# yangsenwxy/VSR

Measured on AMD Instinct MI355X. Metric: voxels/sec fwd+bwd, 4× SR on 16×128×128 cine volumes, 1/2/4/8 MI355X, higher is better.
Workload: dtype bf16

## Files before the change

### vsr_amd/csrc/conv_row.hip

```cpp
#include <cstdlib>
#include "conv_common.h"

namespace {
using namespace vsrk_conv;

constexpr int CR_NW = 8;
constexpr int CR_SEG = 128;
constexpr int CR_SLOT = (CR_SEG + 2) * 128;
constexpr int CR_NSLOT = 4;
constexpr int CR_BIAS = CR_NSLOT * CR_SLOT;
constexpr int CR_LDS = CR_BIAS + 256;
constexpr int CR_MINBAND = 4;
constexpr uint32_t CR_OOB = 0x80000000u;
enum { CE_RES = 1, CE_MASK = 2, CE_ACC = 4, CE_RELU = 8 };

typedef __amdgpu_buffer_rsrc_t CrRsrc;
typedef int cr_v4i __attribute__((ext_vector_type(4)));
__device__ __forceinline__ CrRsrc cr_rsrc(const void* base) {
  const uint64_t b = (uint64_t)base;
  const uint64_t u = ((uint64_t)(uint32_t)__builtin_amdgcn_readfirstlane((int)(uint32_t)(b >> 32)) << 32) |
                     (uint32_t)__builtin_amdgcn_readfirstlane((int)(uint32_t)b);
  return __builtin_amdgcn_make_buffer_rsrc((void*)u, 0, 0x7FFFFFF0, 0x00020000);
}
__device__ __forceinline__ uint4 cr_load16(CrRsrc r, uint32_t voff, uint32_t soff) {
  return __builtin_bit_cast(uint4, __builtin_amdgcn_raw_buffer_load_b128(r, (int)voff, (int)soff, 0));
}
__device__ __forceinline__ void cr_store16(CrRsrc r, uint32_t voff, uint4 v) {
  __builtin_amdgcn_raw_buffer_store_b128(__builtin_bit_cast(cr_v4i, v), r, (int)voff, 0, 0);
}

struct CrView {
  const char* ptr;
  int64_t sn, sd;
  int sh, sw;
};

struct ConvRowArgs {
  CrView x, y, res, msk;
  const void* w;
  const float* bias;
  int cout_pad, cin_pad;
  float out_scale;
  int D, H, W;
  int nseg, nband, band_h, nitems;
};

template <int EM, bool HALO, typename H>
__global__ __launch_bounds__(CR_NW * 64, 1) void conv_row_kernel(ConvRowArgs a) {
  extern __shared__ __attribute__((aligned(16))) char lds[];
  const int tid = threadIdx.x, lane = tid & 63, r = lane & 31, hf = lane >> 5;
  const int wave = __builtin_amdgcn_readfirstlane(tid >> 6);
  const int coh = wave & 1, vq = wave >> 1;

  uint4 wf[9][4];
  {
    const H* wp = reinterpret_cast<const H*>(a.w);
#pragma unroll
    for (int t = 0; t < 9; ++t)
#pragma unroll
      for (int c = 0; c < 4; ++c)
        wf[t][c] = *reinterpret_cast<const uint4*>(wp + ((int64_t)(t * a.cout_pad + coh * 32 + r) * a.cin_pad + c * 16 + 8 * hf));
  }
  const int ecc = 2 * (r >> 4) + hf;
  const int ech = coh * 32 + 8 * ecc;
  const float osc = a.out_scale;
  float* lbias = reinterpret_cast<float*>(lds + CR_BIAS);
  if (tid < 64) lbias[tid] = a.bias ? a.bias[tid] * osc : 0.f;
  if constexpr (!HALO) {
    if (tid < CR_NSLOT * 16)
      *reinterpret_cast<uint4*>(lds + (tid >> 4) * CR_SLOT + ((tid >> 3) & 1) * (CR_SEG + 1) * 128 + (tid & 7) * 16) =
          make_uint4(0, 0, 0, 0);
  }

  uint32_t fa[3], fh[3];
#pragma unroll
  for (int kw = 0; kw < 3; ++kw) {
    const int lv = vq * 32 + r + kw, sz = (lv >> 1) & 7;
    fa[kw] = (uint32_t)(lv * 128 + ((hf ^ (sz & 1)) << 4));
    fh[kw] = (uint32_t)(sz >> 1);
  }
  const int sp = lane & 7;
  constexpr int NSQ = HALO ? 3 : 2;
  const int scol = 8 * wave + (lane >> 3);
  const int hcol = (lane >> 3) == 0 ? -1 : CR_SEG;
  const uint32_t sdst = (uint32_t)((scol + 1) * 128 + ((sp ^ (((scol + 1) >> 1) & 7)) << 4));
  const uint32_t hdst = (uint32_t)((hcol + 1) * 128 + ((sp ^ (((hcol + 1) >> 1) & 7)) << 4));
  const bool halo_lane = wave == 0 && lane < 16;

  f32x16 b0, b1;

  for (int item = blockIdx.x; item < a.nitems; item += gridDim.x) {
    const int band = item % a.nband;
    const int t1 = item / a.nband;
    const int seg = t1 % a.nseg, img = t1 / a.nseg;
    const int in_ = img / a.D, id = img - in_ * a.D;
    const int c0 = seg * CR_SEG;
    const int r0 = band * a.band_h, r1 = min(r0 + a.band_h, a.H);
    const int nstage = r1 - r0 + 1;

    const CrRsrc rx = cr_rsrc(reinterpret_cast<const H*>(a.x.ptr) + (in_ * a.x.sn + id * a.x.sd));
    const CrRsrc ry = cr_rsrc(reinterpret_cast<const H*>(a.y.ptr) + (in_ * a.y.sn + id * a.y.sd));
    const CrRsrc rr = cr_rsrc(reinterpret_cast<const H*>(a.res.ptr) + (in_ * a.res.sn + id * a.res.sd));
    const CrRsrc rm = cr_rsrc(reinterpret_cast<const H*>(a.msk.ptr) + (in_ * a.msk.sn + id * a.msk.sd));

    const uint32_t xcolb = 2u * (uint32_t)((c0 + scol) * a.x.sw + 8 * sp);
    const uint32_t hcolb = 2u * (uint32_t)((c0 + hcol) * a.x.sw + 8 * sp);
    bool xok[3];
    xok[0] = c0 + scol < a.W;
    xok[1] = c0 + scol + 64 < a.W;
    xok[2] = halo_lane && c0 + hcol >= 0 && c0 + hcol < a.W;
    const int ecol = c0 + vq * 32 + (r & 15);
    const uint32_t ycolb = 2u * (uint32_t)(ecol * a.y.sw + ech);
    const uint32_t rcolb = 2u * (uint32_t)(ecol * a.res.sw + ech);
    const uint32_t mcolb = 2u * (uint32_t)(ecol * a.msk.sw + ech);
    const bool yok[2] = {ecol < a.W, ecol + 16 < a.W};

    uint4 stq[CR_NSLOT][NSQ];
    auto load_row = [&](int row, uint4 (&st)[NSQ]) __attribute__((always_inline)) {
      const bool rv = row >= 0 && row < a.H && row <= r1;
      const uint32_t rb = rv ? 2u * (uint32_t)(row * a.x.sh) : 0u;
#pragma unroll
      for (int q = 0; q < 2; ++q) st[q] = cr_load16(rx, (rv && xok[q]) ? xcolb : CR_OOB, rb + 2u * (uint32_t)(64 * q * a.x.sw));
      if constexpr (HALO) st[2] = cr_load16(rx, (rv && xok[2]) ? hcolb : CR_OOB, rb);
    };
    auto write_row = [&](int slot, const uint4 (&st)[NSQ]) __attribute__((always_inline)) {
      char* sl = lds + slot * CR_SLOT;
#pragma unroll
      for (int q = 0; q < 2; ++q) *reinterpret_cast<uint4*>(sl + sdst + q * 64 * 128) = st[q];
      if constexpr (HALO) {
        if (halo_lane) *reinterpret_cast<uint4*>(sl + hdst) = st[NSQ - 1];
      }
    };

    uint4 pr[2], pm[2], po[2];
    auto load_pre = [&](int orow) __attribute__((always_inline)) {
      const bool rv = orow >= r0 && orow < r1;
#pragma unroll
      for (int q = 0; q < 2; ++q) {
        const bool ok = rv && yok[q];
        const int ro = rv ? orow : 0;
        if constexpr (EM & CE_RES) pr[q] = cr_load16(rr, ok ? rcolb : CR_OOB, 2u * (uint32_t)(ro * a.res.sh + 16 * q * a.res.sw));
        if constexpr (EM & CE_MASK) pm[q] = cr_load16(rm, ok ? mcolb : CR_OOB, 2u * (uint32_t)(ro * a.msk.sh + 16 * q * a.msk.sw));
        if constexpr (EM & CE_ACC) po[q] = cr_load16(ry, ok ? ycolb : CR_OOB, 2u * (uint32_t)(ro * a.y.sh + 16 * q * a.y.sw));
      }
    };

    auto flush = [&](const f32x16& A, int orow) __attribute__((always_inline)) {
      const bool rv = orow >= r0 && orow < r1;
      float v[16];
#pragma unroll
      for (int i = 0; i < 16; ++i) v[i] = A[i];
#pragma unroll
      for (int g = 0; g < 4; g += 2) {
#pragma unroll
        for (int i = 0; i < 4; ++i) {
          const auto sw = __builtin_amdgcn_permlane32_swap(__builtin_bit_cast(uint32_t, v[4 * g + i]),
                                                           __builtin_bit_cast(uint32_t, v[4 * g + 4 + i]), false, false);
          v[4 * g + i] = __builtin_bit_cast(float, (uint32_t)sw[0]);
          v[4 * g + 4 + i] = __builtin_bit_cast(float, (uint32_t)sw[1]);
        }
      }
#pragma unroll
      for (int e = 0; e < 8; ++e) {
        const auto sw = __builtin_amdgcn_permlane16_swap(__builtin_bit_cast(uint32_t, v[e]),
                                                         __builtin_bit_cast(uint32_t, v[8 + e]), false, false);
        v[e] = __builtin_bit_cast(float, (uint32_t)sw[0]);
        v[8 + e] = __builtin_bit_cast(float, (uint32_t)sw[1]);
      }
      float bsv[8];
      {
        const float4 c0 = *reinterpret_cast<const float4*>(lbias + ech);
        const float4 c1 = *reinterpret_cast<const float4*>(lbias + ech + 4);
        bsv[0] = c0.x; bsv[1] = c0.y; bsv[2] = c0.z; bsv[3] = c0.w;
        bsv[4] = c1.x; bsv[5] = c1.y; bsv[6] = c1.z; bsv[7] = c1.w;
      }
#pragma unroll
      for (int q = 0; q < 2; ++q) {
        float t[8];
#pragma unroll
        for (int e = 0; e < 8; ++e) {
          t[e] = fmaf(v[8 * q + e], osc, bsv[e]);
          if constexpr (EM & CE_RELU) t[e] = fmaxf(t[e], 0.f);
        }
        if constexpr (EM & CE_MASK) {
          float m[8];
          Chunk<H>::unpack(pm[q], m);
#pragma unroll
          for (int e = 0; e < 8; ++e) t[e] = m[e] > 0.f ? t[e] : 0.f;
        }
        if constexpr (EM & CE_RES) {
          float rs[8];
          Chunk<H>::unpack(pr[q], rs);
#pragma unroll
          for (int e = 0; e < 8; ++e) t[e] += rs[e];
        }
        if constexpr (EM & CE_ACC) {
          float o[8];
          Chunk<H>::unpack(po[q], o);
#pragma unroll
          for (int e = 0; e < 8; ++e) t[e] += o[e];
        }
        const uint32_t yo = ycolb + 2u * (uint32_t)((rv ? orow : 0) * a.y.sh + 16 * q * a.y.sw);
        cr_store16(ry, (rv && yok[q]) ? yo : CR_OOB, Chunk<H>::pack(t));
      }
    };

    __syncthreads();
    load_row(r0 - 1, stq[0]);
    load_row(r0, stq[1]);
    load_row(r0 + 1, stq[2]);
    load_row(r0 + 2, stq[3]);
    write_row(0, stq[0]);
    write_row(1, stq[1]);
    write_row(2, stq[2]);
    load_pre(r0 - 1);

    int s = 0;
    auto step = [&](auto k_c, f32x16& Pcur, const f32x16& Pprev) __attribute__((always_inline)) -> bool {
      constexpr int K = decltype(k_c)::value;
      const int o = r0 + s;
      __syncthreads();
      load_row(o + 3, stq[K]);
      flush(Pprev, o - 1);
      load_pre(o);
#pragma unroll
      for (int kw = 0; kw < 3; ++kw) asm volatile("" : "+v"(fh[kw]));
#pragma unroll
      for (int c = 0; c < 4; ++c) {
#pragma unroll
        for (int kw = 0; kw < 3; ++kw) {
          const uint32_t fo = fa[kw] + (((uint32_t)c ^ fh[kw]) << 5);
#pragma unroll
          for (int kh = 0; kh < 3; ++kh) {
            const uint4 f = *reinterpret_cast<const uint4*>(lds + ((K + kh) % CR_NSLOT) * CR_SLOT + fo);
            if (c == 0 && kw == 0 && kh == 0) {
#pragma unroll
              for (int k = 0; k < 16; ++k) Pcur[k] = 0.f;
            }
            mma<H>(Pcur, wf[kh * 3 + kw][c], f);
          }
        }
      }
      write_row((K + 3) % CR_NSLOT, stq[(K + 3) % CR_NSLOT]);
      return ++s < nstage;
    };
#pragma unroll
    for (int k = 0; k < 16; ++k) b0[k] = b1[k] = 0.f;
    while (step(std::integral_constant<int, 0>{}, b0, b1) && step(std::integral_constant<int, 1>{}, b1, b0) &&
           step(std::integral_constant<int, 2>{}, b0, b1) && step(std::integral_constant<int, 3>{}, b1, b0)) {
    }
  }
}

unsigned long long g_row_launches = 0;

int cr_env_mode() {
  const char* e = getenv("VSRK_CONV_ROW");
  return !e ? -1 : (e[0] == '0' ? 0 : 1);
}
const int g_row_env = cr_env_mode();
int g_row_mode = g_row_env;

int cr_num_cus() {
  static int n = 0;
  if (n == 0) {
    int dev = 0;
    (void)hipGetDevice(&dev);
    if (hipDeviceGetAttribute(&n, hipDeviceAttributeMultiprocessorCount, dev) != hipSuccess || n <= 0) n = 256;
  }
  return n;
}

template <int EM, typename H>
int launch_row(const ConvRowArgs& a, int grid, hipStream_t s) {
  auto kern = a.nseg > 1 ? conv_row_kernel<EM, true, H> : conv_row_kernel<EM, false, H>;
  (void)hipFuncSetAttribute((const void*)kern, hipFuncAttributeMaxDynamicSharedMemorySize, CR_LDS);
  kern<<<grid, CR_NW * 64, CR_LDS, s>>>(a);
  ++g_row_launches;
  VSRK_LAUNCH_CHECK("conv_fwd(row)");
  return VSRK_OK;
}

constexpr bool cr_default_on(int em) {
  return em == 0 || em == CE_RELU || em == CE_RES || em == CE_MASK || em == (CE_RES | CE_ACC);
}

}

extern "C" unsigned long long vsrk_conv_row_launches(void) { return g_row_launches; }

void vsrk_conv_set_row_mode(int mode) { g_row_mode = mode < 0 ? g_row_env : mode; }

int vsrk_conv_fwd_row(const vsrk_conv_desc* d, const vsrk_tensor5* x, const void* w_packed, const float* bias,
                      const vsrk_tensor5* residual, const vsrk_tensor5* mask, const vsrk_tensor5* y, hipStream_t s) {
  if (g_row_mode == 0) return 0;
  if (d->kd != 1 || d->kh != 3 || d->kw != 3 || d->pd != 0 || d->ph != 1 || d->pw != 1) return 0;
  if (x->c != 64 || y->c != 64 || x->shuffle > 1 || y->shuffle > 1) return 0;
  if (d->prologue || d->mask_slope || d->bias_perm_r > 1 || d->subpixel) return 0;
  if (d->act != VSRK_ACT_NONE && d->act != VSRK_ACT_RELU) return 0;
  if (x->n != y->n || x->d != y->d || x->h != y->h || x->w != y->w) return 0;
  const int em = (residual ? CE_RES : 0) | (mask ? CE_MASK : 0) | (d->accumulate ? CE_ACC : 0) |
                 (d->act == VSRK_ACT_RELU ? CE_RELU : 0);
  if (em != 0 && em != CE_RELU && em != CE_RES && em != CE_MASK && em != (CE_RES | CE_ACC)) return 0;
  if (g_row_mode < 0 && !cr_default_on(em)) return 0;
  if (!chunk_ok(x, 2)) return 0;
  for (const vsrk_tensor5* t : {x, y, residual, mask}) {
    if (!t) continue;
    const int64_t span = (int64_t)(t->h - 1) * t->sh + (int64_t)(t->w - 1) * t->sw + 64;
    if (t->sn < 0 || t->sd < 0 || t->sh < 0 || t->sw < 0 || 2 * span >= 0x7FFFFFF0ll) return 0;
    if (t->sh >= (1ll << 30) || t->sw >= (1ll << 30)) return 0;
  }
  const int64_t nimg = (int64_t)y->n * y->d;
  if (nimg == 0 || y->h == 0 || y->w == 0) return 1;
  auto view = [](const vsrk_tensor5* t) {
    CrView v;
    v.ptr = (const char*)t->ptr;
    v.sn = t->sn; v.sd = t->sd; v.sh = (int)t->sh; v.sw = (int)t->sw;
    return v;
  };
  ConvRowArgs a;
  a.x = view(x);
  a.y = view(y);
  a.res = view(residual ? residual : y);
  a.msk = view(mask ? mask : y);
  a.w = w_packed;
  a.bias = bias;
  a.cin_pad = round_up(x->c, 32);
  a.cout_pad = round_up(y->c, 128);
  a.out_scale = d->out_scale;
  a.D = y->d; a.H = y->h; a.W = y->w;
  a.nseg = ceil_div(y->w, CR_SEG);
  const int64_t target = vsrk_capped_grid(cr_num_cus());
  const int64_t cols = nimg * a.nseg;
  int64_t nb = std::max<int64_t>(1, std::min<int64_t>(ceil_div64(target, cols), y->h));
  a.band_h = (int)std::max<int64_t>(ceil_div64(y->h, nb), std::min(CR_MINBAND, y->h));
  a.nband = ceil_div(y->h, a.band_h);
  const int64_t nitems = cols * a.nband;
  if (nitems >= (1ll << 31)) return 0;
  a.nitems = (int)nitems;
  const int grid = (int)vsrk_capped_grid(std::min<int64_t>(nitems, cr_num_cus()));
  int rc = vsrk_dispatch16(x->dtype, [&](auto tag) {
    using H = decltype(tag);
    switch (em) {
      case 0: return launch_row<0, H>(a, grid, s);
      case CE_RELU: return launch_row<CE_RELU, H>(a, grid, s);
      case CE_RES: return launch_row<CE_RES, H>(a, grid, s);
      case CE_MASK: return launch_row<CE_MASK, H>(a, grid, s);
      default: return launch_row<CE_RES | CE_ACC, H>(a, grid, s);
    }
  });
  return rc == VSRK_OK ? 1 : -rc;
}
```

### vsr_amd/csrc/conv_wgrad_row.hip

```cpp
#include <algorithm>
#include <cstdlib>
#include "conv_common.h"

namespace {
using namespace vsrk_conv;

constexpr int RW_NW = 8;
constexpr int RW_KC = 4;
constexpr int RW_SEG = 32 * RW_KC;
constexpr int RW_XV = RW_SEG + 8;
constexpr int RW_XP = RW_XV / 8;
constexpr int RW_YP = RW_SEG / 8;
constexpr int RW_NP = RW_XP + RW_YP;
constexpr int RW_NQ = (RW_NP + RW_NW - 1) / RW_NW;
constexpr int RW_XSLOT = RW_XP * 1024;
constexpr int RW_YSLOT = RW_YP * 1024;
constexpr int RW_NXS = 4, RW_NYS = 2;
constexpr int RW_YBASE = RW_NXS * RW_XSLOT;
constexpr int RW_LDS = RW_YBASE + RW_NYS * RW_YSLOT;
constexpr int RW_COW = 64;
constexpr int RW_SLAB = 9 * RW_COW * 64 + RW_COW;
constexpr uint32_t RW_OOB = 0x80000000u;

#ifndef RW_ABL
#define RW_ABL 0
#endif

__host__ __device__ constexpr int rw_swz(int j) { return 2 * ((j >> 1) & 1) + 4 * ((j >> 3) & 1); }

typedef __amdgpu_buffer_rsrc_t RwRsrc;
__device__ __forceinline__ RwRsrc rw_rsrc(const void* base) {
  const uint64_t b = (uint64_t)base;
  const uint64_t u = ((uint64_t)(uint32_t)__builtin_amdgcn_readfirstlane((int)(uint32_t)(b >> 32)) << 32) |
                     (uint32_t)__builtin_amdgcn_readfirstlane((int)(uint32_t)b);
  return __builtin_amdgcn_make_buffer_rsrc((void*)u, 0, 0x7FFFFFF0, 0x00020000);
}
typedef uint32_t rw_u32x4 __attribute__((ext_vector_type(4)));
__device__ __forceinline__ void rw_st16(uint32_t addr, uint4 v) {
  *(__attribute__((address_space(3))) rw_u32x4*)(size_t)addr = __builtin_bit_cast(rw_u32x4, v);
}

typedef float f32x4_t __attribute__((ext_vector_type(4)));
template <typename H> struct V8R;
template <> struct V8R<bf16> { typedef bf16x8 type; };
template <> struct V8R<f16> { typedef f16x8 type; };
__device__ __forceinline__ f32x4_t rw_mfma(bf16x8 a, bf16x8 b, f32x4_t c) {
  return __builtin_amdgcn_mfma_f32_16x16x32_bf16(a, b, c, 0, 0, 0);
}
__device__ __forceinline__ f32x4_t rw_mfma(f16x8 a, f16x8 b, f32x4_t c) {
  return __builtin_amdgcn_mfma_f32_16x16x32_f16(a, b, c, 0, 0, 0);
}
__device__ __forceinline__ uint4 rw_frag(uint32_t p0, uint32_t p1) {
  const v4i16 a = __builtin_amdgcn_ds_read_tr16_b64_v4i16((lds_v4i16*)(size_t)p0);
  const v4i16 b = __builtin_amdgcn_ds_read_tr16_b64_v4i16((lds_v4i16*)(size_t)p1);
  return __builtin_bit_cast(uint4, __builtin_shufflevector(a, b, 0, 1, 2, 3, 4, 5, 6, 7));
}

constexpr int RW_MAXB = 16;

struct RowArgs {
  const char* x;
  const char* dy;
  int xoff[RW_MAXB], yoff[RW_MAXB];
  uint16_t tapm[RW_MAXB];
  int tapm_x;
  float* ws;
  int64_t xsn, xsd, xsh, xsw, ysn, ysd, ysh, ysw;
  int xd, H, W;
  int bands, band_h, nseg, ncot, ncic, nsplit;
  int want_bias;
  int prio;
};

template <typename H, bool SPM>
__global__ __launch_bounds__(RW_NW * 64, 1) void wgrad_row_kernel(RowArgs a) {
  using V8 = typename V8R<H>::type;
  extern __shared__ __attribute__((aligned(16))) char lds[];
  const int lane = threadIdx.x & 63;
  const int wave = __builtin_amdgcn_readfirstlane(threadIdx.x >> 6);
  const int coh = wave & 1, cib = wave >> 1;

  const int ncombo = a.ncot * a.ncic;
  const int L = xcd_remap(blockIdx.x, a.nsplit * ncombo);
  const int split = L / ncombo;
  const int combo = L - split * ncombo;
  const int cot = combo % a.ncot, cic = combo / a.ncot;
  const int seg = split % a.nseg;
  const int t0 = split / a.nseg;
  const int band = t0 % a.bands, img = t0 / a.bands;
  const int nb = img / a.xd, dd = img - nb * a.xd;
  const int h0 = band * a.band_h;
  const int nst = min(a.H, h0 + a.band_h) - h0;
  const int w0 = seg * RW_SEG;
  const unsigned tapm = SPM ? (unsigned)a.tapm[a.tapm_x ? cic : cot] : 0x1ffu;
  const char* xim = a.x + 2 * (nb * a.xsn + dd * a.xsd + a.xoff[cic]);
  const char* yim = a.dy + 2 * (nb * a.ysn + dd * a.ysd + a.yoff[cot]);

  static_assert(RW_XP == 2 * RW_NW + 1 && RW_YP == 2 * RW_NW, "piece roles");
  uint32_t goff[RW_NQ], loff[RW_NQ];
#pragma unroll
  for (int q = 0; q < RW_NQ; ++q) {
    const bool isx = q != 2 && q != 3;
    const int j = q == 4 ? 2 * RW_NW : wave + RW_NW * (q & 1);
    if (isx) {
      const int v = 8 * j + (lane >> 3);
      const int col = w0 - 1 + v;
      const bool ok = v < RW_SEG + 2 && col >= 0 && col < a.W;
      goff[q] = ok ? (uint32_t)(2 * (col * (int)a.xsw + 8 * (lane & 7))) : RW_OOB;
      loff[q] = (uint32_t)(j * 1024 + (lane >> 3) * 128 + 16 * ((lane & 7) ^ rw_swz(v)));
    } else {
      const int v = 8 * j + (lane >> 3);
      const int col = w0 + v;
      goff[q] = col < a.W ? (uint32_t)(2 * (col * (int)a.ysw + 8 * (lane & 7))) : RW_OOB;
      loff[q] = (uint32_t)(j * 1024 + (lane >> 3) * 128 + 16 * ((lane & 7) ^ rw_swz(v)));
    }
  }
  const uint32_t lbase = lds_addr(lds);
  auto load_set = [&](int t, uint4 (&r)[RW_NQ]) __attribute__((always_inline)) {
    const int xr = h0 - 1 + t;
    const bool xok = xr >= 0 && xr < a.H;
    const int yr = t - 2;
    const bool yok = yr >= 0 && yr < nst;
    const RwRsrc rx = rw_rsrc(xim + 2 * (int64_t)(xok ? xr : 0) * a.xsh);
    const RwRsrc ry = rw_rsrc(yim + 2 * (int64_t)(h0 + (yok ? yr : 0)) * a.ysh);
#pragma unroll
    for (int q = 0; q < RW_NQ; ++q) {
      const bool isx = q != 2 && q != 3;
      if (q == 4 && wave != 0) break;
      r[q] = __builtin_bit_cast(uint4, __builtin_amdgcn_raw_buffer_load_b128(
                                           isx ? rx : ry, (int)((isx ? xok : yok) ? goff[q] : RW_OOB), 0, 0));
    }
  };
  auto store_set = [&](int t, const uint4 (&r)[RW_NQ]) __attribute__((always_inline)) {
    const uint32_t xs = lbase + (uint32_t)(t % RW_NXS) * RW_XSLOT;
    const int yr = t - 2;
    const uint32_t ys = lbase + RW_YBASE + (uint32_t)((yr < 0 ? 0 : yr) % RW_NYS) * RW_YSLOT;
#pragma unroll
    for (int q = 0; q < RW_NQ; ++q) {
      const bool isx = q != 2 && q != 3;
      if (q == 4 && wave != 0) break;
      if (isx) rw_st16(xs + loff[q], r[q]);
      else if (yr >= 0) rw_st16(ys + loff[q], r[q]);
    }
  };

  const int g = lane >> 4, qq = (lane >> 2) & 3, pp = lane & 3;
  uint32_t xo[3][2];
#pragma unroll
  for (int kw = 0; kw < 3; ++kw)
#pragma unroll
    for (int h = 0; h < 2; ++h) {
      const int v = kw + 8 * g + qq + 4 * h;
      xo[kw][h] = (uint32_t)(v * 128 + 16 * ((2 * cib + (pp >> 1)) ^ rw_swz(v)) + 8 * (pp & 1));
    }
  uint32_t yo[2][2];
#pragma unroll
  for (int b = 0; b < 2; ++b)
#pragma unroll
    for (int h = 0; h < 2; ++h) {
      const int v = 8 * g + qq + 4 * h;
      yo[b][h] = (uint32_t)(v * 128 + 16 * ((2 * (2 * coh + b) + (pp >> 1)) ^ rw_swz(v)) + 8 * (pp & 1));
    }

  f32x4_t acc[3][3][2];
#pragma unroll
  for (int i = 0; i < 18; ++i) acc[i / 6][(i / 2) % 3][i % 2] = f32x4_t{0.f, 0.f, 0.f, 0.f};
  f32x4_t bacc[2] = {f32x4_t{0.f, 0.f, 0.f, 0.f}, f32x4_t{0.f, 0.f, 0.f, 0.f}};
  uint4 ones;
  {
    const H one = from_f32<H>(1.f);
    const uint16_t u = __builtin_bit_cast(uint16_t, one);
    const uint32_t w2 = (uint32_t)u | ((uint32_t)u << 16);
    ones = make_uint4(w2, w2, w2, w2);
  }

  const int last = nst + 1;
  uint4 stg[RW_NQ], stg2[RW_NQ];
  load_set(0, stg);
  if (1 <= last) load_set(1, stg2);
  store_set(0, stg);
  if (1 <= last) store_set(1, stg2);
  if (2 <= last) {
    load_set(2, stg);
    store_set(2, stg);
  }
  __syncthreads();
  if (3 <= last) load_set(3, stg);
  __builtin_amdgcn_sched_barrier(0);

  for (int s = 0; s < nst; ++s) {
    uint32_t xa[3][3][2], ya[2][2];
#pragma unroll
    for (int kh = 0; kh < 3; ++kh) {
      const uint32_t xrow = lbase + (uint32_t)((s + kh) % RW_NXS) * RW_XSLOT;
#pragma unroll
      for (int kw = 0; kw < 3; ++kw)
#pragma unroll
        for (int h = 0; h < 2; ++h) {
          xa[kh][kw][h] = xrow + xo[kw][h];
          asm volatile("" : "+v"(xa[kh][kw][h]));
        }
    }
    {
      const uint32_t yr = lbase + RW_YBASE + (uint32_t)(s % RW_NYS) * RW_YSLOT;
#pragma unroll
      for (int b = 0; b < 2; ++b)
#pragma unroll
        for (int h = 0; h < 2; ++h) {
          ya[b][h] = yr + yo[b][h];
          asm volatile("" : "+v"(ya[b][h]));
        }
    }
    uint4 xf[2][3], yf[2][2];
    auto load_group = [&](int G) __attribute__((always_inline)) {
      const int kc = G / 3, kh = G % 3;
      if (kh == 0) {
#pragma unroll
        for (int b = 0; b < 2; ++b) yf[kc & 1][b] = rw_frag(ya[b][0] + kc * 4096, ya[b][1] + kc * 4096);
      }
#pragma unroll
      for (int kw = 0; kw < 3; ++kw) xf[G & 1][kw] = rw_frag(xa[kh][kw][0] + kc * 4096, xa[kh][kw][1] + kc * 4096);
    };
    load_group(0);
#pragma unroll
    for (int G = 0; G < 3 * RW_KC; ++G) {
      if (G + 1 < 3 * RW_KC) load_group(G + 1);
      __builtin_amdgcn_sched_barrier(0);
      if (a.prio) __builtin_amdgcn_s_setprio(1);
      const int kc = G / 3, kh = G % 3;
#pragma unroll
      for (int kw = 0; kw < 3; ++kw) {
        if (SPM && !((tapm >> (kh * 3 + kw)) & 1)) continue;
#pragma unroll
        for (int b = 0; b < 2; ++b)
          if (RW_ABL & 2) acc[kh][kw][b][0] += __builtin_bit_cast(float, yf[kc & 1][b].x ^ xf[G & 1][kw].y);
          else acc[kh][kw][b] = rw_mfma(__builtin_bit_cast(V8, yf[kc & 1][b]), __builtin_bit_cast(V8, xf[G & 1][kw]),
                                   acc[kh][kw][b]);
      }
      if (kh == 1 && kc == cib) {
#pragma unroll
        for (int b = 0; b < 2; ++b)
          bacc[b] = rw_mfma(__builtin_bit_cast(V8, yf[kc & 1][b]), __builtin_bit_cast(V8, ones), bacc[b]);
      }
      if (a.prio) __builtin_amdgcn_s_setprio(0);
      __builtin_amdgcn_sched_barrier(0);
    }
    if (!(RW_ABL & 1)) {
      if (s + 3 <= last) store_set(s + 3, stg);
      asm volatile("s_waitcnt lgkmcnt(0)\n\ts_barrier" ::: "memory");
      if (s + 4 <= last) load_set(s + 4, stg);
    }
    __builtin_amdgcn_sched_barrier(0);
  }

  float* out = a.ws + ((int64_t)split * ncombo + combo) * RW_SLAB;
  const int l15 = lane & 15, lg = lane >> 4;
#pragma unroll
  for (int t9 = 0; t9 < 9; ++t9)
#pragma unroll
    for (int b = 0; b < 2; ++b)
#pragma unroll
      for (int i = 0; i < 4; ++i) {
        const int co = 32 * coh + 16 * b + 4 * lg + i, ci = 16 * cib + l15;
        out[(t9 * RW_COW + co) * 64 + ci] = ((tapm >> t9) & 1) ? acc[t9 / 3][t9 % 3][b][i] : 0.f;
      }
  if (a.want_bias && cic == 0) {
    float* part = reinterpret_cast<float*>(lds);
    __syncthreads();
    if (l15 == 0) {
#pragma unroll
      for (int b = 0; b < 2; ++b)
#pragma unroll
        for (int i = 0; i < 4; ++i) part[cib * 64 + 32 * coh + 16 * b + 4 * lg + i] = bacc[b][i];
    }
    __syncthreads();
    if (threadIdx.x < RW_COW) {
      const int c = threadIdx.x;
      out[9 * RW_COW * 64 + c] = ((part[c] + part[64 + c]) + part[128 + c]) + part[192 + c];
    }
  }
}

int g_wrow_mode = -1;

int wrow_num_cus() {
  static int n = 0;
  if (n == 0) {
    int dev = 0;
    (void)hipGetDevice(&dev);
    if (hipDeviceGetAttribute(&n, hipDeviceAttributeMultiprocessorCount, dev) != hipSuccess || n <= 0) n = 256;
  }
  return n;
}

}

void vsrk_conv_set_wgrad_row_mode(int mode) { g_wrow_mode = mode; }

bool vsrk_wgrad_row_plan(const vsrk_conv_desc* d, const vsrk_tensor5* x, const vsrk_tensor5* dy, VsrkRowPlan* p) {
  if (g_wrow_mode < 0) {
    const char* e = getenv("VSRK_WGRAD_ROW");
    g_wrow_mode = (e && e[0] == '0') ? 0 : 1;
  }
  if (g_wrow_mode == 0) return false;
  if (!vsrk_is16(x->dtype) || dy->dtype != x->dtype) return false;
  if (d->kd != 1 || d->kh != 3 || d->kw != 3 || d->pd != 0 || d->ph != 1 || d->pw != 1) return false;
  if (d->prologue != VSRK_PRO_NONE) return false;
  if (x->c % 64 || dy->c % 64 || (x->shuffle > 1 && dy->shuffle > 1)) return false;
  if (d->subpixel && (x->shuffle > 1 || dy->shuffle > 1) && g_wrow_mode != 2) return false;
  if (x->c / 64 > RW_MAXB || dy->c / 64 > RW_MAXB) return false;
  for (const vsrk_tensor5* t : {x, dy}) {
    if (t->shuffle <= 1) continue;
    const int r = t->shuffle, cph = t->c / (r * r);
    if (cph * r * r != t->c || cph % 64) return false;
  }
  if (x->n != dy->n || x->d != dy->d || x->h != dy->h || x->w != dy->w) return false;
  if (!chunk_ok(x, 2) || !chunk_ok(dy, 2)) return false;
  for (const vsrk_tensor5* t : {x, dy}) {
    const int64_t r = t->shuffle > 1 ? t->shuffle : 1;
    if (t->sn < 0 || t->sd < 0 || t->sh < 0 || t->sw < 0 ||
        (int64_t)(RW_XV + 2) * r * t->sw + (r - 1) * t->sh + t->c >= (1ll << 29))
      return false;
  }
  const int64_t images = (int64_t)x->n * x->d;
  if (images <= 0 || x->h <= 0 || x->w <= 0) return false;
  const int nseg = ceil_div(x->w, RW_SEG);
  const int ncot = dy->c / RW_COW, ncic = x->c / 64;
  const int64_t per_band = images * nseg * ncot * ncic;
  int64_t want = std::max<int64_t>(1, wrow_num_cus());
  if (vsrk_g_grid_cap > 0) want = std::min<int64_t>(want, vsrk_g_grid_cap);
  int bands = (int)std::max<int64_t>(1, std::min<int64_t>((want + per_band / 2) / per_band, ceil_div(x->h, 8)));
  {
    static int ov = -1;
    if (ov < 0) {
      const char* e = getenv("VSRK_WGRAD_ROW_BANDS");
      ov = e ? std::max(0, atoi(e)) : 0;
    }
    if (ov > 0) bands = std::min(ov, x->h);
  }
  if (vsrk_g_grid_cap > 0) bands = std::max(1, std::min(bands, x->h));
  p->band_h = ceil_div(x->h, bands);
  p->bands = ceil_div(x->h, p->band_h);
  p->nseg = nseg;
  p->ncot = ncot;
  p->ncic = ncic;
  const int64_t ns = images * p->bands * nseg;
  if (ns * ncot * ncic >= (1ll << 30)) return false;
  p->nsplit = (int)ns;
  p->cot_w = RW_COW;
  p->slab = RW_SLAB;
  p->ws_bytes = (size_t)ns * ncot * ncic * RW_SLAB * sizeof(float);
  return true;
}

int vsrk_conv_wgrad_row(const vsrk_conv_desc* d, const vsrk_tensor5* x, const vsrk_tensor5* dy, int want_bias,
                        float* ws, size_t ws_bytes, VsrkRowPlan* plan, hipStream_t s) {
  VsrkRowPlan p;
  if (!vsrk_wgrad_row_plan(d, x, dy, &p)) return 0;
  if (ws_bytes < p.ws_bytes) return 0;
  RowArgs a;
  a.x = (const char*)x->ptr;
  a.dy = (const char*)dy->ptr;
  a.ws = ws;
  auto blocks = [](const vsrk_tensor5* t, int64_t& sh, int64_t& sw, int* off) {
    const int r = t->shuffle > 1 ? t->shuffle : 1;
    sh = (int64_t)r * t->sh;
    sw = (int64_t)r * t->sw;
    const int cph = t->c / (r * r);
    for (int b = 0; b < t->c / 64; ++b) {
      const int c = 64 * b, sub = c / cph, cc = c - sub * cph;
      off[b] = (int)((sub / r) * t->sh + (sub % r) * t->sw + cc);
    }
  };
  a.xsn = x->sn; a.xsd = x->sd;
  a.ysn = dy->sn; a.ysd = dy->sd;
  blocks(x, a.xsh, a.xsw, a.xoff);
  blocks(dy, a.ysh, a.ysw, a.yoff);
  const vsrk_tensor5* spt = x->shuffle > 1 ? x : (dy->shuffle > 1 ? dy : nullptr);
  const bool spm = d->subpixel && spt;
  a.tapm_x = spt == x;
  if (spm) {
    const int r = spt->shuffle, cph = spt->c / (r * r);
    const int32_t code = d->subpixel & ~(1 << 25);
    for (int b = 0; b < spt->c / 64; ++b) a.tapm[b] = (uint16_t)subpixel_tapmask(code, r, 64 * b / cph);
  }
  a.xd = x->d;
  a.H = x->h;
  a.W = x->w;
  a.bands = p.bands;
  a.band_h = p.band_h;
  a.nseg = p.nseg;
  a.ncot = p.ncot;
  a.ncic = p.ncic;
  a.nsplit = p.nsplit;
  a.want_bias = want_bias;
  {
    static int prio = -1;
    if (prio < 0) {
      const char* e = getenv("VSRK_WGRAD_ROW_PRIO");
      prio = (e && e[0] == '1') ? 1 : 0;
    }
    a.prio = prio;
  }
  const int grid = p.nsplit * p.ncot * p.ncic;
  vsrk_dispatch16(x->dtype, [&](auto tag) {
    using H = decltype(tag);
    auto kern = spm ? wgrad_row_kernel<H, true> : wgrad_row_kernel<H, false>;
    (void)hipFuncSetAttribute((const void*)kern, hipFuncAttributeMaxDynamicSharedMemorySize, RW_LDS);
    kern<<<grid, RW_NW * 64, RW_LDS, s>>>(a);
    return 0;
  });
  *plan = p;
  return 1;
}
```

Before: 61.82 million.

## Interleave epilogue flush with MFMA groups and prefetch LDS reads one group ahead

Splits the previous row's epilogue (permlane swaps, bias, store) into four parts and interleaves them between groups of MFMA instructions, with sched_barriers, for non-halo, non-residual variants. LDS fragment reads are grouped in threes and issued one group ahead of the MFMAs that consume them, so LDS latency and epilogue work overlap with matrix math. It also adds ROW_ABL ablation macros, which are off by default. The costs are higher register pressure from the extra fragment buffers, and sched_barriers that may block the compiler's own better schedules.

After: 62.12 million (median of 3 runs). No clear change (+0.5%).

```diff
diff --git a/vsr_amd/csrc/conv_row.hip b/vsr_amd/csrc/conv_row.hip
--- a/vsr_amd/csrc/conv_row.hip
+++ b/vsr_amd/csrc/conv_row.hip
@@ -13,6 +13,14 @@
 constexpr int CR_MINBAND = 4;
 constexpr uint32_t CR_OOB = 0x80000000u;
 enum { CE_RES = 1, CE_MASK = 2, CE_ACC = 4, CE_RELU = 8 };
+
+#ifndef ROW_ABL
+#define ROW_ABL 0
+#endif
+
+constexpr int CR_AHEAD = 1;
+constexpr int CR_FLUSH_AT[4] = {0, 2, 4, 6};
+constexpr bool cr_spread(int em, bool halo) { return !halo && (em == 0 || em == CE_RELU); }
 
 typedef __amdgpu_buffer_rsrc_t CrRsrc;
 typedef int cr_v4i __attribute__((ext_vector_type(4)));
@@ -133,49 +141,53 @@
     };
 
     uint4 pr[2], pm[2], po[2];
-    auto load_pre = [&](int orow) __attribute__((always_inline)) {
+    auto load_pre = [&](int orow, int q) __attribute__((always_inline)) {
       const bool rv = orow >= r0 && orow < r1;
-#pragma unroll
-      for (int q = 0; q < 2; ++q) {
-        const bool ok = rv && yok[q];
-        const int ro = rv ? orow : 0;
-        if constexpr (EM & CE_RES) pr[q] = cr_load16(rr, ok ? rcolb : CR_OOB, 2u * (uint32_t)(ro * a.res.sh + 16 * q * a.res.sw));
-        if constexpr (EM & CE_MASK) pm[q] = cr_load16(rm, ok ? mcolb : CR_OOB, 2u * (uint32_t)(ro * a.msk.sh + 16 * q * a.msk.sw));
-        if constexpr (EM & CE_ACC) po[q] = cr_load16(ry, ok ? ycolb : CR_OOB, 2u * (uint32_t)(ro * a.y.sh + 16 * q * a.y.sw));
+      const bool ok = rv && yok[q];
+      const int ro = rv ? orow : 0;
+      if constexpr (EM & CE_RES) pr[q] = cr_load16(rr, ok ? rcolb : CR_OOB, 2u * (uint32_t)(ro * a.res.sh + 16 * q * a.res.sw));
+      if constexpr (EM & CE_MASK) pm[q] = cr_load16(rm, ok ? mcolb : CR_OOB, 2u * (uint32_t)(ro * a.msk.sh + 16 * q * a.msk.sw));
+      if constexpr (EM & CE_ACC) po[q] = cr_load16(ry, ok ? ycolb : CR_OOB, 2u * (uint32_t)(ro * a.y.sh + 16 * q * a.y.sw));
+    };
+
+    auto flush_part = [&](auto part_c, float (&v)[16], float (&bsv)[8], const f32x16& A, int orow)
+                          __attribute__((always_inline)) {
+      constexpr int PART = decltype(part_c)::value;
+      if constexpr ((ROW_ABL & 1) != 0) {
+        if constexpr (PART == 0) {
+#pragma unroll
+          for (int i = 0; i < 16; ++i) asm volatile("" ::"v"(A[i]));
+        }
+        return;
       }
-    };
-
-    auto flush = [&](const f32x16& A, int orow) __attribute__((always_inline)) {
-      const bool rv = orow >= r0 && orow < r1;
-      float v[16];
-#pragma unroll
-      for (int i = 0; i < 16; ++i) v[i] = A[i];
-#pragma unroll
-      for (int g = 0; g < 4; g += 2) {
-#pragma unroll
-        for (int i = 0; i < 4; ++i) {
-          const auto sw = __builtin_amdgcn_permlane32_swap(__builtin_bit_cast(uint32_t, v[4 * g + i]),
-                                                           __builtin_bit_cast(uint32_t, v[4 * g + 4 + i]), false, false);
-          v[4 * g + i] = __builtin_bit_cast(float, (uint32_t)sw[0]);
-          v[4 * g + 4 + i] = __builtin_bit_cast(float, (uint32_t)sw[1]);
-        }
-      }
-#pragma unroll
-      for (int e = 0; e < 8; ++e) {
-        const auto sw = __builtin_amdgcn_permlane16_swap(__builtin_bit_cast(uint32_t, v[e]),
-                                                         __builtin_bit_cast(uint32_t, v[8 + e]), false, false);
-        v[e] = __builtin_bit_cast(float, (uint32_t)sw[0]);
-        v[8 + e] = __builtin_bit_cast(float, (uint32_t)sw[1]);
-      }
-      float bsv[8];
-      {
+      if constexpr (PART == 0) {
+#pragma unroll
+        for (int i = 0; i < 16; ++i) v[i] = A[i];
+#pragma unroll
+        for (int g = 0; g < 4; g += 2) {
+#pragma unroll
+          for (int i = 0; i < 4; ++i) {
+            const auto sw = __builtin_amdgcn_permlane32_swap(__builtin_bit_cast(uint32_t, v[4 * g + i]),
+                                                             __builtin_bit_cast(uint32_t, v[4 * g + 4 + i]), false, false);
+            v[4 * g + i] = __builtin_bit_cast(float, (uint32_t)sw[0]);
+            v[4 * g + 4 + i] = __builtin_bit_cast(float, (uint32_t)sw[1]);
+          }
+        }
+      } else if constexpr (PART == 1) {
+#pragma unroll
+        for (int e = 0; e < 8; ++e) {
+          const auto sw = __builtin_amdgcn_permlane16_swap(__builtin_bit_cast(uint32_t, v[e]),
+                                                           __builtin_bit_cast(uint32_t, v[8 + e]), false, false);
+          v[e] = __builtin_bit_cast(float, (uint32_t)sw[0]);
+          v[8 + e] = __builtin_bit_cast(float, (uint32_t)sw[1]);
+        }
         const float4 c0 = *reinterpret_cast<const float4*>(lbias + ech);
         const float4 c1 = *reinterpret_cast<const float4*>(lbias + ech + 4);
         bsv[0] = c0.x; bsv[1] = c0.y; bsv[2] = c0.z; bsv[3] = c0.w;
         bsv[4] = c1.x; bsv[5] = c1.y; bsv[6] = c1.z; bsv[7] = c1.w;
-      }
-#pragma unroll
-      for (int q = 0; q < 2; ++q) {
+      } else {
+        constexpr int q = PART - 2;
+        const bool rv = orow >= r0 && orow < r1;
         float t[8];
 #pragma unroll
         for (int e = 0; e < 8; ++e) {
@@ -203,6 +215,13 @@
         const uint32_t yo = ycolb + 2u * (uint32_t)((rv ? orow : 0) * a.y.sh + 16 * q * a.y.sw);
         cr_store16(ry, (rv && yok[q]) ? yo : CR_OOB, Chunk<H>::pack(t));
       }
+    };
+    auto flush = [&](const f32x16& A, int orow) __attribute__((always_inline)) {
+      float v[16], bsv[8];
+      flush_part(std::integral_constant<int, 0>{}, v, bsv, A, orow);
+      flush_part(std::integral_constant<int, 1>{}, v, bsv, A, orow);
+      flush_part(std::integral_constant<int, 2>{}, v, bsv, A, orow);
+      flush_part(std::integral_constant<int, 3>{}, v, bsv, A, orow);
     };
 
     __syncthreads();
@@ -213,35 +232,63 @@
     write_row(0, stq[0]);
     write_row(1, stq[1]);
     write_row(2, stq[2]);
-    load_pre(r0 - 1);
+    load_pre(r0 - 1, 0);
+    load_pre(r0 - 1, 1);
 
     int s = 0;
     auto step = [&](auto k_c, f32x16& Pcur, const f32x16& Pprev) __attribute__((always_inline)) -> bool {
       constexpr int K = decltype(k_c)::value;
+      constexpr bool SPREAD = cr_spread(EM, HALO);
+      constexpr int D = SPREAD ? CR_AHEAD : 0, GS = 3, NG = 36 / GS;
       const int o = r0 + s;
       __syncthreads();
-      load_row(o + 3, stq[K]);
-      flush(Pprev, o - 1);
-      load_pre(o);
+      if constexpr (!(ROW_ABL & 4)) load_row(o + 3, stq[K]);
+      float v[16], bsv[8];
+      if constexpr (!SPREAD) {
+        flush(Pprev, o - 1);
+        load_pre(o, 0);
+        load_pre(o, 1);
+      }
 #pragma unroll
       for (int kw = 0; kw < 3; ++kw) asm volatile("" : "+v"(fh[kw]));
-#pragma unroll
-      for (int c = 0; c < 4; ++c) {
-#pragma unroll
-        for (int kw = 0; kw < 3; ++kw) {
+      uint4 fr[D + 1][GS];
+      auto read_group = [&](int g) __attribute__((always_inline)) {
+#pragma unroll
+        for (int j = 0; j < GS; ++j) {
+          const int m = g * GS + j, c = m / 9, kw = (m / 3) % 3, kh = m % 3;
           const uint32_t fo = fa[kw] + (((uint32_t)c ^ fh[kw]) << 5);
-#pragma unroll
-          for (int kh = 0; kh < 3; ++kh) {
-            const uint4 f = *reinterpret_cast<const uint4*>(lds + ((K + kh) % CR_NSLOT) * CR_SLOT + fo);
-            if (c == 0 && kw == 0 && kh == 0) {
-#pragma unroll
-              for (int k = 0; k < 16; ++k) Pcur[k] = 0.f;
-            }
-            mma<H>(Pcur, wf[kh * 3 + kw][c], f);
+          fr[g % (D + 1)][j] = *reinterpret_cast<const uint4*>(lds + ((K + kh) % CR_NSLOT) * CR_SLOT + fo);
+        }
+      };
+#pragma unroll
+      for (int g = 0; g < D; ++g) read_group(g);
+#pragma unroll
+      for (int k = 0; k < 16; ++k) Pcur[k] = 0.f;
+#pragma unroll
+      for (int g = 0; g < NG; ++g) {
+        if (g + D < NG) read_group(g + D);
+        if constexpr (SPREAD) {
+          __builtin_amdgcn_sched_barrier(0);
+          if (g == CR_FLUSH_AT[0]) flush_part(std::integral_constant<int, 0>{}, v, bsv, Pprev, o - 1);
+          if (g == CR_FLUSH_AT[1]) flush_part(std::integral_constant<int, 1>{}, v, bsv, Pprev, o - 1);
+          if (g == CR_FLUSH_AT[2]) {
+            flush_part(std::integral_constant<int, 2>{}, v, bsv, Pprev, o - 1);
+            load_pre(o, 0);
           }
-        }
+          if (g == CR_FLUSH_AT[3]) {
+            flush_part(std::integral_constant<int, 3>{}, v, bsv, Pprev, o - 1);
+            load_pre(o, 1);
+          }
+        }
+#pragma unroll
+        for (int j = 0; j < GS; ++j) {
+          const int m = g * GS + j, c = m / 9, kw = (m / 3) % 3, kh = m % 3;
+          if constexpr ((ROW_ABL & 2) != 0) Pcur[kh] += __builtin_bit_cast(float, fr[g % (D + 1)][j].x ^ wf[kh * 3 + kw][c].y);
+          else mma<H>(Pcur, wf[kh * 3 + kw][c], fr[g % (D + 1)][j]);
+        }
+        if constexpr (SPREAD) __builtin_amdgcn_sched_barrier(0);
       }
-      write_row((K + 3) % CR_NSLOT, stq[(K + 3) % CR_NSLOT]);
+      if constexpr (!(ROW_ABL & 4)) write_row((K + 3) % CR_NSLOT, stq[(K + 3) % CR_NSLOT]);
       return ++s < nstage;
     };
 #pragma unroll
```

## Stagger conv row flush across waves and shorten epilogue with register bias

Applied to the files above, without the earlier changes.

In the row convolution kernel, the upper four waves now flush their current output row right after its MMAs instead of flushing the previous row at the start of the next stage. This spreads epilogue stores and MMA work across waves, and is enabled only for the epilogue forms picked by a compile-time mask. Bias values are loaded straight into registers instead of staged through LDS, and output is packed with vector bf16/f16 conversions. The wgrad priority toggle changes from a runtime env var to a compile-time macro, which removes a kernel argument and the getenv check.

Measured after the change: 62.45 million before, 63.18 million after (median of 4 runs). Within noise of the previous version (+1.2%).

```diff
diff --git a/vsr_amd/csrc/conv_row.hip b/vsr_amd/csrc/conv_row.hip
--- a/vsr_amd/csrc/conv_row.hip
+++ b/vsr_amd/csrc/conv_row.hip
@@ -8,11 +8,35 @@
 constexpr int CR_SEG = 128;
 constexpr int CR_SLOT = (CR_SEG + 2) * 128;
 constexpr int CR_NSLOT = 4;
-constexpr int CR_BIAS = CR_NSLOT * CR_SLOT;
-constexpr int CR_LDS = CR_BIAS + 256;
 constexpr int CR_MINBAND = 4;
 constexpr uint32_t CR_OOB = 0x80000000u;
 enum { CE_RES = 1, CE_MASK = 2, CE_ACC = 4, CE_RELU = 8 };
+
+#ifndef CR_SHORT_FLUSH
+#define CR_SHORT_FLUSH 1
+#endif
+#ifndef CR_STAGGER
+#define CR_STAGGER 0x0c
+#endif
+constexpr int CR_BIAS = CR_NSLOT * CR_SLOT;
+constexpr int CR_LDS = CR_BIAS + (CR_SHORT_FLUSH ? 0 : 256);
+
+typedef __bf16 cr_bf16x2 __attribute__((ext_vector_type(2)));
+typedef _Float16 cr_f16x2 __attribute__((ext_vector_type(2)));
+template <typename H> struct CrV2;
+template <> struct CrV2<bf16> { typedef cr_bf16x2 type; };
+template <> struct CrV2<f16> { typedef cr_f16x2 type; };
+template <typename H>
+__device__ __forceinline__ uint4 cr_pack(const float* t) {
+  if (!CR_SHORT_FLUSH) return Chunk<H>::pack(t);
+  uint32_t u[4];
+#pragma unroll
+  for (int i = 0; i < 4; ++i) {
+    const typename CrV2<H>::type p = {(H)t[2 * i], (H)t[2 * i + 1]};
+    u[i] = __builtin_bit_cast(uint32_t, p);
+  }
+  return make_uint4(u[0], u[1], u[2], u[3]);
+}
 
 typedef __amdgpu_buffer_rsrc_t CrRsrc;
 typedef int cr_v4i __attribute__((ext_vector_type(4)));
@@ -45,12 +69,13 @@
   int nseg, nband, band_h, nitems;
 };
 
-template <int EM, bool HALO, typename H>
+template <int EM, bool HALO, bool STG, typename H>
 __global__ __launch_bounds__(CR_NW * 64, 1) void conv_row_kernel(ConvRowArgs a) {
   extern __shared__ __attribute__((aligned(16))) char lds[];
   const int tid = threadIdx.x, lane = tid & 63, r = lane & 31, hf = lane >> 5;
   const int wave = __builtin_amdgcn_readfirstlane(tid >> 6);
   const int coh = wave & 1, vq = wave >> 1;
+  const bool late = STG && wave >= 4;
 
   uint4 wf[9][4];
   {
@@ -64,8 +89,14 @@
   const int ecc = 2 * (r >> 4) + hf;
   const int ech = coh * 32 + 8 * ecc;
   const float osc = a.out_scale;
+#if CR_SHORT_FLUSH
+  float bsv[8];
+#pragma unroll
+  for (int e = 0; e < 8; ++e) bsv[e] = a.bias ? a.bias[ech + e] * osc : 0.f;
+#else
   float* lbias = reinterpret_cast<float*>(lds + CR_BIAS);
   if (tid < 64) lbias[tid] = a.bias ? a.bias[tid] * osc : 0.f;
+#endif
   if constexpr (!HALO) {
     if (tid < CR_NSLOT * 16)
       *reinterpret_cast<uint4*>(lds + (tid >> 4) * CR_SLOT + ((tid >> 3) & 1) * (CR_SEG + 1) * 128 + (tid & 7) * 16) =
@@ -167,6 +198,7 @@
         v[e] = __builtin_bit_cast(float, (uint32_t)sw[0]);
         v[8 + e] = __builtin_bit_cast(float, (uint32_t)sw[1]);
       }
+#if !CR_SHORT_FLUSH
       float bsv[8];
       {
         const float4 c0 = *reinterpret_cast<const float4*>(lbias + ech);
@@ -174,6 +206,7 @@
         bsv[0] = c0.x; bsv[1] = c0.y; bsv[2] = c0.z; bsv[3] = c0.w;
         bsv[4] = c1.x; bsv[5] = c1.y; bsv[6] = c1.z; bsv[7] = c1.w;
       }
+#endif
 #pragma unroll
       for (int q = 0; q < 2; ++q) {
         float t[8];
@@ -201,7 +234,7 @@
           for (int e = 0; e < 8; ++e) t[e] += o[e];
         }
         const uint32_t yo = ycolb + 2u * (uint32_t)((rv ? orow : 0) * a.y.sh + 16 * q * a.y.sw);
-        cr_store16(ry, (rv && yok[q]) ? yo : CR_OOB, Chunk<H>::pack(t));
+        cr_store16(ry, (rv && yok[q]) ? yo : CR_OOB, cr_pack<H>(t));
       }
     };
 
@@ -221,7 +254,7 @@
       const int o = r0 + s;
       __syncthreads();
       load_row(o + 3, stq[K]);
-      flush(Pprev, o - 1);
+      if (!late) flush(Pprev, o - 1);
       load_pre(o);
 #pragma unroll
       for (int kw = 0; kw < 3; ++kw) asm volatile("" : "+v"(fh[kw]));
@@ -241,6 +274,7 @@
           }
         }
       }
+      if (late) flush(Pcur, o);
       write_row((K + 3) % CR_NSLOT, stq[(K + 3) % CR_NSLOT]);
       return ++s < nstage;
     };
@@ -273,7 +307,9 @@
 
 template <int EM, typename H>
 int launch_row(const ConvRowArgs& a, int grid, hipStream_t s) {
-  auto kern = a.nseg > 1 ? conv_row_kernel<EM, true, H> : conv_row_kernel<EM, false, H>;
+  constexpr int form = EM == 0 ? 0 : EM == CE_RELU ? 1 : EM == CE_RES ? 2 : EM == CE_MASK ? 3 : 4;
+  constexpr bool STG = (CR_STAGGER >> form) & 1;
+  auto kern = a.nseg > 1 ? conv_row_kernel<EM, true, STG, H> : conv_row_kernel<EM, false, STG, H>;
   (void)hipFuncSetAttribute((const void*)kern, hipFuncAttributeMaxDynamicSharedMemorySize, CR_LDS);
   kern<<<grid, CR_NW * 64, CR_LDS, s>>>(a);
   ++g_row_launches;
diff --git a/vsr_amd/csrc/conv_wgrad_row.hip b/vsr_amd/csrc/conv_wgrad_row.hip
--- a/vsr_amd/csrc/conv_wgrad_row.hip
+++ b/vsr_amd/csrc/conv_wgrad_row.hip
@@ -25,6 +25,9 @@
 #ifndef RW_ABL
 #define RW_ABL 0
 #endif
+#ifndef RW_PRIO
+#define RW_PRIO 0
+#endif
 
 __host__ __device__ constexpr int rw_swz(int j) { return 2 * ((j >> 1) & 1) + 4 * ((j >> 3) & 1); }
 
@@ -69,7 +72,6 @@
   int xd, H, W;
   int bands, band_h, nseg, ncot, ncic, nsplit;
   int want_bias;
-  int prio;
 };
 
 template <typename H, bool SPM>
@@ -226,7 +228,7 @@
     for (int G = 0; G < 3 * RW_KC; ++G) {
       if (G + 1 < 3 * RW_KC) load_group(G + 1);
       __builtin_amdgcn_sched_barrier(0);
-      if (a.prio) __builtin_amdgcn_s_setprio(1);
+      if (RW_PRIO) __builtin_amdgcn_s_setprio(1);
       const int kc = G / 3, kh = G % 3;
 #pragma unroll
       for (int kw = 0; kw < 3; ++kw) {
@@ -242,7 +244,7 @@
         for (int b = 0; b < 2; ++b)
           bacc[b] = rw_mfma(__builtin_bit_cast(V8, yf[kc & 1][b]), __builtin_bit_cast(V8, ones), bacc[b]);
       }
-      if (a.prio) __builtin_amdgcn_s_setprio(0);
+      if (RW_PRIO) __builtin_amdgcn_s_setprio(0);
       __builtin_amdgcn_sched_barrier(0);
     }
     if (!(RW_ABL & 1)) {
@@ -394,14 +396,6 @@
   a.ncic = p.ncic;
   a.nsplit = p.nsplit;
   a.want_bias = want_bias;
-  {
-    static int prio = -1;
-    if (prio < 0) {
-      const char* e = getenv("VSRK_WGRAD_ROW_PRIO");
-      prio = (e && e[0] == '1') ? 1 : 0;
-    }
-    a.prio = prio;
-  }
   const int grid = p.nsplit * p.ncot * p.ncic;
   vsrk_dispatch16(x->dtype, [&](auto tag) {
     using H = decltype(tag);
```
